# jianfch/stable-ts

Measured on AMD Instinct MI355X. Metric: real-time factor (audio-sec/wall-sec) large-v3 word_timestamps=True, higher is better.
Workload: dtype f16; 1 GPU; large-v3 (random-init, weight recipe BENCH_WEIGHTS = the parity-pinned recipe of tests/test_gpu_f16_depth.py), 10 min synthetic 16 kHz audio per GPU, word_timestamps=True, beam_size=5, 112 decode steps/window, window-parallel batch 20, default regrouping inside the timed pass; mode=transcribe, windows_per_gpu=20, segments=125, words=1670, parallelism=dp1 (windows sharded, no data-path collective)

## Files before the change

stable_ts_amd/csrc/swx_gemm.hip:

```cpp
#include <cstdlib>
#include <type_traits>
#include <array>
#include <vector>
#include <cstdio>
#include "swx_common.h"
#include "swx_kernels.h"

namespace {

template <typename T>
__device__ __forceinline__ void epilogue_store(const GemmArgs &g, int row, int col, float v)
{
    if (row >= g.M || col >= g.N) return;
    if (g.epi & EPI_BIAS) v += g.bias[col];
    if (g.epi & EPI_GELU) v = gelu_erf(v);
    if (g.epi & EPI_RESF32MOD) v += g.Rf[(size_t)(row % g.res_mod) * g.N + col];
    if (g.epi & EPI_RES) v += to_f32<T>(((const T *)g.R)[(size_t)row * g.ldr + col]);
    if (g.epi & EPI_STORE_VT) {
        const int w = row / g.vt_s, sidx = row - w * g.vt_s;
        ((T *)g.C)[(size_t)w * g.vt_bs + (size_t)col * g.vt_kp + sidx] = from_f32<T>(v);
    } else if (g.epi & EPI_CBATCH) {
        const int w = row / g.vt_s, sidx = row - w * g.vt_s;
        ((T *)g.C)[(size_t)w * g.vt_bs + (size_t)sidx * g.ldc + col] = from_f32<T>(v);
    } else if (g.epi & EPI_OUT_F32) ((float *)g.C)[(size_t)row * g.ldc + col] = v;
// ... 471 lines not shown
    for (int e = 0; e < 8; ++e) bv[e] = ((g.epi & EPI_BIAS) && gn + e < g.N) ? g.bias[gn + e] : 0.f;
#pragma unroll
    for (int p = 0; p < 4; ++p) {
        f16x8 rv[4];
        if (g.epi & EPI_RES) {
#pragma unroll
            for (int it = 0; it < 4; ++it) {
                const int gm = m0 + p * 64 + it * 16 + rb;
                rv[it] = (gm < g.M && full) ? *(const f16x8 *)((const f16 *)g.R + (size_t)gm * g.ldr + gn) : (f16x8)(f16)0;
            }
        }
        if (wm == (p >> 1)) {
#pragma unroll
            for (int ii = 0; ii < 4; ++ii)
#pragma unroll
                for (int j = 0; j < 4; ++j)
#pragma unroll
                    for (int r = 0; r < 4; ++r) Cs[ii * 16 + row_l + r][wn * 64 + j * 16 + col_l] = acc[(p & 1) * 4 + ii][j][r];
        }
        __syncthreads();
#pragma unroll
        for (int it = 0; it < 4; ++it) {
            const int row = it * 16 + rb, gm = m0 + p * 64 + row;
            if (gm >= g.M || !col_ok) continue;
            const f32x4 lo = *(const f32x4 *)&Cs[row][c8], hi = *(const f32x4 *)&Cs[row][c8 + 4];
            float v[8] = {lo[0], lo[1], lo[2], lo[3], hi[0], hi[1], hi[2], hi[3]};
#pragma unroll
            for (int e = 0; e < 8; ++e) v[e] += bv[e];
            if (g.epi & EPI_GELU) {
                gelu_erf_n<8>(v);
            }
            f16 *cp = (f16 *)g.C + (size_t)gm * g.ldc + gn;
            if (full) {
                if (g.epi & EPI_RES) {
#pragma unroll
                    for (int e = 0; e < 8; ++e) v[e] += (float)rv[it][e];
                }
                f16x8 o;
#pragma unroll
                for (int e = 0; e < 8; ++e) o[e] = (f16)v[e];
                *(f16x8 *)cp = o;
            } else {
                for (int e = 0; e < 8 && gn + e < g.N; ++e) {
                    float t = v[e];
                    if (g.epi & EPI_RES) t += (float)((const f16 *)g.R)[(size_t)gm * g.ldr + gn + e];
                    cp[e] = (f16)t;
                }
            }
        }
        if (p < 3) __syncthreads();
    }
}

constexpr int B8_HALF = 128 * 128;
constexpr int B8_BUF = 4 * B8_HALF;

template <int N>
__device__ __forceinline__ void b8_wait_vm()
{
    asm volatile("s_waitcnt vmcnt(%0)" ::"n"(N) : "memory");
}
__device__ __forceinline__ void b8_barrier()
{
    asm volatile("s_barrier" ::: "memory");
}
__device__ __forceinline__ void b8_wait_lds()
{
    asm volatile("s_waitcnt lgkmcnt(0)" ::: "memory");
}

__global__ __launch_bounds__(512) void gemm_f16_big8(GemmArgs g)
{
    extern __shared__ __attribute__((aligned(1024))) unsigned char ring[];
    const int tid = threadIdx.x, lane = tid & 63, wave = tid >> 6;
    const int wave_u = __builtin_amdgcn_readfirstlane(wave);
    const int wm = wave >> 2, wn = wave & 3;
    const int wm_u = wave_u >> 2;
    int bx = blockIdx.x, by = blockIdx.y;
    {
        const int gx = gridDim.x, gy = gridDim.y, nwg = gx * gy, orig = by * gx + bx;
        const int xcd = orig & 7, q = nwg >> 3, r = nwg & 7;
        const int wg = (xcd < r ? xcd * (q + 1) : r * (q + 1) + (xcd - r) * q) + (orig >> 3);
        if (g.tile_order != 1 || gx <= 4) { bx = wg % gx; by = wg / gx; }
        else {
            constexpr int GN = 4;
            const int nfull = gx / GN, per = GN * gy;
            const int grp = wg / per;
            if (grp < nfull) { const int rem = wg - grp * per; by = rem / GN; bx = grp * GN + (rem - by * GN); }
            else { const int gl = gx - nfull * GN, rem = wg - nfull * per; by = rem / gl; bx = nfull * GN + (rem - by * gl); }
        }
    }
    const int m0 = by * BG, n0 = bx * BG;
    const f16 *A = (const f16 *)g.A;
    const f16 *W = (const f16 *)g.W;

    f32x4 acc[8][4];
#pragma unroll
    for (int i = 0; i < 8; ++i)
#pragma unroll
        for (int j = 0; j < 4; ++j) acc[i][j] = (f32x4){0.f, 0.f, 0.f, 0.f};

    const f16 *sA[2][2], *sB[2][2];
#pragma unroll
    for (int h = 0; h < 2; ++h)
#pragma unroll
        for (int c = 0; c < 2; ++c) {
            const int lr = (wave * 2 + c) * 8 + (lane >> 3);
            const int slot = (lane & 7) ^ ((lr >> 1) & 7);
            const int ra = (lr >> 6) * 128 + h * 64 + (lr & 63);
            const int rb = (lr >> 5) * 64 + h * 32 + (lr & 31);
            const int gm = m0 + ra < g.M ? m0 + ra : g.M - 1;
            const int gn = n0 + rb < g.N ? n0 + rb : g.N - 1;
            sA[h][c] = A + (size_t)gm * g.lda + slot * 8;
            sB[h][c] = W + (size_t)gn * g.ldw + slot * 8;
        }
    typedef __attribute__((address_space(3))) void lds_void;
    const unsigned ring0 = (unsigned)(uintptr_t)(lds_void *)ring;
    auto issue = [&](int kt, auto which_c) {
        constexpr int which = decltype(which_c)::value;
        constexpr bool isA = which == 0 || which == 3;
        constexpr int h = which >= 2 ? 1 : 0;
        constexpr int off = (isA ? 0 : 2 * B8_HALF) + h * B8_HALF;
        const unsigned dst = ring0 + (kt & 1) * B8_BUF + off + wave_u * 2048;
#pragma unroll
// ... 29 lines not shown
        constexpr int ih = decltype(ih_c)::value, jh = decltype(jh_c)::value;
        __builtin_amdgcn_s_setprio(1);
#pragma unroll
        for (int kk = 0; kk < 2; ++kk)
#pragma unroll
            for (int i = 0; i < 4; ++i)
#pragma unroll
                for (int j = 0; j < 2; ++j)
                    acc[ih * 4 + i][jh * 2 + j] = __builtin_amdgcn_mfma_f32_16x16x32_f16(fa[i][kk], fb[j][kk], acc[ih * 4 + i][jh * 2 + j], 0, 0, 0);
        __builtin_amdgcn_s_setprio(0);
    };
    auto tile = [&](auto mode_c, int t) {
        constexpr int MODE = decltype(mode_c)::value;
        const int buf = t & 1;
        read_a(buf, 0);
        read_b(buf, 0, fb0);
        b8_wait_vm<MODE == 2 ? 2 : 8>();
        b8_barrier();
        b8_wait_lds();
        if (MODE < 2) issue(t + 1, I3());
        quad(I0(), I0(), fb0);
        b8_barrier();
        read_b(buf, 1, fb1);
        b8_wait_vm<MODE == 2 ? 0 : 8>();
        b8_barrier();
        b8_wait_lds();
        if (MODE == 0) issue(t + 2, I0());
        quad(I0(), I1(), fb1);
        b8_barrier();
        read_a(buf, 1);
        b8_barrier();
        b8_wait_lds();
        if (MODE == 0) issue(t + 2, I1());
        quad(I1(), I1(), fb1);
        b8_barrier();
        if (MODE == 0) b8_wait_vm<8>();
        if (MODE == 1) b8_wait_vm<4>();
        b8_barrier();
        if (MODE == 0) issue(t + 2, I2());
        quad(I1(), I0(), fb0);
        b8_barrier();
    };

    issue(0, I0()); issue(0, I1()); issue(0, I2()); issue(0, I3());
    issue(1, I0()); issue(1, I1()); issue(1, I2());
    b8_wait_vm<10>();
    b8_barrier();
    if (wm_u == 1) b8_barrier();
    int t = 0;
    for (; t < KT - 2; ++t) tile(I0(), t);
    tile(I1(), t);
    tile(I2(), t + 1);
    if (wm_u == 0) b8_barrier();
    big_tile_epilogue(g, ring, acc, m0, n0, tid, lane, wm, wn);
}

constexpr int BK32 = 16, LD32 = BK32 + 1;

template <int BMT, int BNT, int ST>
__global__ __launch_bounds__(256) void gemm_f32_tiled(GemmArgs g)
{
    constexpr int WN = BNT >= 128 ? 2 : 1, WM = 4 / WN;
    constexpr int WROWS = BMT / WM, WCOLS = BNT / WN;
    constexpr int NI = WROWS / 16, NJ = WCOLS / 16;
    constexpr int NA = (BMT * 4 + 255) / 256, NB = (BNT * 4 + 255) / 256;
    static_assert(NI >= 1 && NJ >= 1, "a wave owns at least one 16 x 16 fragment");
    __shared__ float As[2][BMT][LD32];
    __shared__ float Bs[2][BNT][LD32];
    const int tid = threadIdx.x, lane = tid & 63, wave = tid >> 6;
    const int wm = WN == 2 ? wave >> 1 : wave, wn = WN == 2 ? wave & 1 : 0;
    const int m0 = blockIdx.y * BMT, n0 = blockIdx.x * BNT;
    const float *A = (const float *)g.A;
    const float *W = (const float *)g.W;

    f32x4 acc[NI][NJ];
#pragma unroll
    for (int i = 0; i < NI; ++i)
#pragma unroll
        for (int j = 0; j < NJ; ++j) acc[i][j] = (f32x4){0.f, 0.f, 0.f, 0.f};

    f32x4 ra[ST][NA], rb[ST][NB];
    auto load_regs = [&](int st, int k0) {
#pragma unroll
        for (int i = 0; i < NA; ++i) {
            const int c = tid + 256 * i, row = c >> 2, kc = (c & 3) * 4;
            const int gm = m0 + row;
            ra[st][i] = (row < BMT && gm < g.M) ? *(const f32x4 *)(A + (size_t)gm * g.lda + k0 + kc) : (f32x4){0.f, 0.f, 0.f, 0.f};
        }
#pragma unroll
        for (int i = 0; i < NB; ++i) {
            const int c = tid + 256 * i, row = c >> 2, kc = (c & 3) * 4;
            const int gn = n0 + row;
            rb[st][i] = (row < BNT && gn < g.N) ? *(const f32x4 *)(W + (size_t)gn * g.ldw + k0 + kc) : (f32x4){0.f, 0.f, 0.f, 0.f};
        }
    };
    auto store_lds = [&](int st, int buf) {
#pragma unroll
        for (int i = 0; i < NA; ++i) {
            const int c = tid + 256 * i, row = c >> 2, kc = (c & 3) * 4;
            if (row < BMT) {
#pragma unroll
                for (int e = 0; e < 4; ++e) As[buf][row][kc + e] = ra[st][i][e];
            }
        }
#pragma unroll
        for (int i = 0; i < NB; ++i) {
            const int c = tid + 256 * i, row = c >> 2, kc = (c & 3) * 4;
            if (row < BNT) {
// ... 191 lines not shown
        const int m = t * 16 + fr;
        aok[t] = m < g.M;
        ap[t] = A + (size_t)(aok[t] ? m : 0) * g.lda + kb + fk;
    }
    f16x8 af[2][MT];
#pragma unroll
    for (int t = 0; t < MT; ++t) { const f16x8 v = *(const f16x8 *)(ap[t]); af[0][t] = aok[t] ? v : zero8; }
#pragma unroll
    for (int ks = 0; ks < NKS_MAX; ++ks) {
        if (ks < nks) {
            if (ks + 1 < nks) {
#pragma unroll
                for (int t = 0; t < MT; ++t) { const f16x8 v = *(const f16x8 *)(ap[t] + (ks + 1) * 32); af[(ks + 1) & 1][t] = aok[t] ? v : zero8; }
            }
#pragma unroll
            for (int t = 0; t < MT; ++t) acc[t] = __builtin_amdgcn_mfma_f32_16x16x32_f16(af[ks & 1][t], wf[ks], acc[t], 0, 0, 0);
        }
    }

    if (wave > 0) {
#pragma unroll
        for (int t = 0; t < MT; ++t) red[wave - 1][t][lane] = acc[t];
    }
    __syncthreads();
    if (wave == 0) {
        const int col = n0 + (lane & 15), row_l = (lane >> 4) * 4;
#pragma unroll
        for (int t = 0; t < MT; ++t) {
            f32x4 v = acc[t];
#pragma unroll
            for (int w = 0; w < 3; ++w) {
                const f32x4 o = red[w][t][lane];
                v[0] += o[0]; v[1] += o[1]; v[2] += o[2]; v[3] += o[3];
            }
#pragma unroll
            for (int r = 0; r < 4; ++r) epilogue_store<f16>(g, t * 16 + row_l + r, col, v[r]);
        }
    }
}

}

int swx_gemm_plan_f16(int M, int N, int K, int epi, int64_t ldc, int64_t ldr, bool ptr16, int force_kernel, int flags)
{
    if (K % 32 != 0) return -4;
    const bool skinny_ok = M <= 128 && K % 128 == 0 && K / 128 <= 10 && N <= 16384;
    if (force_kernel == 2) return skinny_ok ? SWX_GEMM_SKINNY : -4;
    if (skinny_ok && force_kernel != 1 && force_kernel < 7) return SWX_GEMM_SKINNY;
    const bool glds_ok = K % 64 == 0 && ptr16;
    if (force_kernel >= 7 && !glds_ok) return -4;
    if (force_kernel == 1 || !glds_ok) return SWX_GEMM_TILED_REG;
    const int64_t t128 = (int64_t)cdiv(N, BN) * cdiv(M, BM);
    const bool narrow = force_kernel == 8 || (force_kernel != 9 && N % 64 == 0 && t128 < 224);
    const bool big_ok = !(epi & ~(EPI_BIAS | EPI_GELU | EPI_RES)) && ldc % 8 == 0 && (!(epi & EPI_RES) || ldr % 8 == 0);
    if (force_kernel == 12) return big_ok && K >= 128 ? SWX_GEMM_BIG : -4;
    const int64_t t256 = (int64_t)cdiv(M, BG) * cdiv(N, BG);
    const double fill = (double)t256 / (double)(((t256 + 255) / 256) * 256);
    if (force_kernel == 0 && big_ok && t256 >= 200 && K >= 512 && (fill >= 0.9 || (fill >= 0.75 && K >= 2560)) &&
        !(flags & SWX_FLAG_NO_BIG_TILE))
        return SWX_GEMM_BIG;
    const bool ring_ok = K >= 128;
    if (force_kernel == 10 || force_kernel == 11) return !ring_ok ? -4 : force_kernel == 10 ? SWX_GEMM_RING64 : SWX_GEMM_RING128;
    if (force_kernel == 0 && ring_ok && M > 256 && (narrow || t128 <= 256) && !(flags & SWX_FLAG_NO_RING))
        return narrow ? SWX_GEMM_RING64 : SWX_GEMM_RING128;
    return narrow ? SWX_GEMM_GLDS64 : SWX_GEMM_GLDS128;
}

int swx_gemm(int dtype, const GemmArgs &g, int force_kernel, hipStream_t s)
{
    if (g.M <= 0 || g.N <= 0) return 0;
    if (dtype == SWX_F16) {
        if (g.lda % 8 != 0 || g.ldw % 8 != 0) return -4;
        const bool ptr16 = (uintptr_t)g.A % 16 == 0 && (uintptr_t)g.W % 16 == 0;
        const bool cr16 = (uintptr_t)g.C % 16 == 0 && (!(g.epi & EPI_RES) || (uintptr_t)g.R % 16 == 0);
        const int plan = swx_gemm_plan_f16(g.M, g.N, g.K, g.epi, cr16 ? g.ldc : 1, cr16 ? g.ldr : 1, ptr16, force_kernel, swx_flags());
        if (plan < 0) return plan;
        if (plan == SWX_GEMM_SKINNY) {
            SwxProfScope prof(PC_GEMM_SKINNY, 2.0 * ((double)g.N * g.K + (double)g.M * g.K) + (double)g.M * g.N * ((g.epi & EPI_OUT_F32) ? 4 : 2), s);
            dim3 grid(cdiv(g.N, 16));
            const int mt = cdiv(g.M, 16);
            switch (mt) {
                case 1: hipLaunchKernelGGL(gemm_f16_skinny<1>, grid, dim3(256), 0, s, g); break;
                case 2: hipLaunchKernelGGL(gemm_f16_skinny<2>, grid, dim3(256), 0, s, g); break;
                case 3: hipLaunchKernelGGL(gemm_f16_skinny<3>, grid, dim3(256), 0, s, g); break;
                case 4: hipLaunchKernelGGL(gemm_f16_skinny<4>, grid, dim3(256), 0, s, g); break;
                case 5: hipLaunchKernelGGL(gemm_f16_skinny<5>, grid, dim3(256), 0, s, g); break;
                case 6: hipLaunchKernelGGL(gemm_f16_skinny<6>, grid, dim3(256), 0, s, g); break;
                case 7: hipLaunchKernelGGL(gemm_f16_skinny<7>, grid, dim3(256), 0, s, g); break;
                default: hipLaunchKernelGGL(gemm_f16_skinny<8>, grid, dim3(256), 0, s, g); break;
            }
        } else {
            SwxProfScope prof(PC_GEMM_TILED, 2.0 * (double)g.M * g.N * g.K, s);
            const dim3 grid(cdiv(g.N, BN), cdiv(g.M, BM));
            switch (plan) {
                case SWX_GEMM_BIG: {
                    GemmArgs gb = g;
                    gb.tile_order = (swx_flags() & SWX_FLAG_BIG8_GROUPED) ? 1 : 0;
                    hipLaunchKernelGGL(gemm_f16_big8, dim3(cdiv(g.N, BG), cdiv(g.M, BG)), dim3(512), 2 * B8_BUF, s, gb); break;
                }
                case SWX_GEMM_RING64: launch_ring<64, 3>(g, s); break;
                case SWX_GEMM_RING128: launch_ring<128, 3>(g, s); break;
                case SWX_GEMM_GLDS64: hipLaunchKernelGGL(gemm_f16_glds_64, dim3(cdiv(g.N, 64), grid.y), dim3(256), 0, s, g); break;
                case SWX_GEMM_GLDS128: hipLaunchKernelGGL(gemm_f16_glds_128, grid, dim3(256), 0, s, g); break;
                default: hipLaunchKernelGGL(gemm_f16_tiled, grid, dim3(256), 0, s, g); break;
            }
        }
    } else {
        if (g.K % 16 != 0 || g.lda % 4 != 0 || g.ldw % 4 != 0) return -4;
        SwxProfScope prof(PC_GEMM_TILED, 2.0 * (double)g.M * g.N * g.K, s);
        if (g.M <= BM && g.N >= 256 && g.K % 64 == 0 && force_kernel != 8) {
            if (g.N >= 2560) hipLaunchKernelGGL((gemm_f32_rows64<2>), dim3(cdiv(g.N, 32), cdiv(g.M, 64)), dim3(256), 0, s, g);
            else hipLaunchKernelGGL((gemm_f32_rows64<1>), dim3(cdiv(g.N, 16), cdiv(g.M, 64)), dim3(256), 0, s, g);
        } else if (g.M <= BM && g.N >= 256) {
            if (g.N >= 2560) hipLaunchKernelGGL((gemm_f32_tiled<64, 32, 4>), dim3(cdiv(g.N, 32), cdiv(g.M, 64)), dim3(256), 0, s, g);
            else hipLaunchKernelGGL((gemm_f32_tiled<64, 16, 4>), dim3(cdiv(g.N, 16), cdiv(g.M, 64)), dim3(256), 0, s, g);
        } else {
            hipLaunchKernelGGL((gemm_f32_tiled<128, 128, 4>), dim3(cdiv(g.N, BN), cdiv(g.M, BM)), dim3(256), 0, s, g);
        }
    }
    SWX_CHECK_LAUNCH();
    return 0;
}
```

stable_ts_amd/csrc/swx_kernels.h:

```cpp
#pragma once
#include <hip/hip_runtime.h>
#include <stdint.h>
#include "../../include/swx.h"

#define EPI_BIAS 1
#define EPI_GELU 2
#define EPI_RES 4
#define EPI_OUT_F32 8
#define EPI_RESF32MOD 16
#define EPI_CBATCH 64
#define EPI_STORE_VT 32
#define EPI_KV 128

#define EPI_QKV_VT 256

struct GemmArgs {
    const void *A; int64_t lda;
    const void *W; int64_t ldw;
    const float *bias;
    const void *R; int64_t ldr;
    const float *Rf; int res_mod;
    void *C; int64_t ldc;
    void *C2;
    void *P; int64_t p_bs;
    int p_nkpad, p_vcol0;
    int M, N, K;
    int epi;
    int vt_s, vt_kp; int64_t vt_bs;
    int vt_zero_pad;
    int tile_order;
};
int swx_gemm(int dtype, const GemmArgs &g, int force_kernel, hipStream_t s);
enum { SWX_GEMM_TILED_REG = 0, SWX_GEMM_SKINNY = 1, SWX_GEMM_GLDS128 = 2, SWX_GEMM_GLDS64 = 3, SWX_GEMM_RING64 = 4, SWX_GEMM_RING128 = 5,
       SWX_GEMM_BIG = 6 };
int swx_gemm_plan_f16(int M, int N, int K, int epi, int64_t ldc, int64_t ldr, bool ptr16, int force_kernel, int flags);

#define SWX_FLAG_TABLE(X) \
    X(NO_FAST_STEP, 0)         \
    X(KCACHE_CHUNKED, 1)       \
    X(SELFATTN_NO_DEEP, 2)     \
    X(DEC_NO_W1, 4)            \
    X(TALL_NO_W8, 5)           \
    X(FLASH_NO_QB1, 6)         \
    X(XKV_PACK_SEPARATE, 7)    \
    X(SELFATTN_NO_MQ, 8)       \
    X(XQ_FULL_TILE, 9)         \
    X(DEC_W1_FULL_TILE, 10)    \
    X(NO_PACKED_XKV, 11)       \
    X(SELECT_MEM, 13)          \
    X(NO_GRAPH, 14)            \
    X(NO_PREFETCH, 15)         \
    X(NO_RING, 16)             \
    X(NO_BIG_TILE, 17)         \
    X(SCORE_TILED, 18)         \
    X(NO_TALL, 19)             \
    X(NO_FUSED_XQ, 20)         \
    X(TICKET, 21)              \
    X(BIG8_GROUPED, 22)        \
    X(XKV_TWO_LAUNCHES, 23)    \
    X(LOUDNESS_ONE_WG, 24)     \
    X(XATTN_R5, 25)            \
    X(FLASH_PIPELINED, 26)     \
    X(SELFATTN_WG5, 27)        \
    X(QKV_SEPARATE_VT, 28)
#define SWX_FLAG_DEFINE(name, bit) constexpr int SWX_FLAG_##name = 1 << (bit);
SWX_FLAG_TABLE(SWX_FLAG_DEFINE)
#undef SWX_FLAG_DEFINE
#define SWX_FLAG_IN_RANGE(name, bit) && (bit) >= 0 && (bit) <= 30
#define SWX_FLAG_OR(name, bit) | (int64_t(1) << (bit))
#define SWX_FLAG_SUM(name, bit) + (int64_t(1) << (bit))
static_assert(true SWX_FLAG_TABLE(SWX_FLAG_IN_RANGE), "SWX_FLAG_TABLE: a bit index outside 0..30");
static_assert((int64_t(0) SWX_FLAG_TABLE(SWX_FLAG_OR)) == (int64_t(0) SWX_FLAG_TABLE(SWX_FLAG_SUM)), "SWX_FLAG_TABLE: two switches share a bit");
#undef SWX_FLAG_IN_RANGE
#undef SWX_FLAG_OR
#undef SWX_FLAG_SUM
#define SWX_DEFAULT_FLAGS 0
int swx_flags();

struct KLayout { int sp, sh, sc; };
__host__ __device__ inline KLayout swx_klayout(int chunked, int n_ctx, int d)
{
    return chunked ? KLayout{8, 64 * n_ctx, 8 * n_ctx} : KLayout{d, 64, 8};
}
__host__ __device__ inline int swx_kidx(const KLayout &L, int pos, int h, int chunk) { return h * L.sh + chunk * L.sc + pos * L.sp; }

#define DEC_LN 1
#define DEC_GELU 2
#define DEC_RES 4
#define DEC_QKV 8
#define DEC_SLAB 16
#define DEC_TICKET 32
struct DecPrefetch {
    const void *base;
    int lines;
};
DecPrefetch swx_dec_prefetch_of(const void *packed_w, int M, int N, int K, int epi);

struct DecGemmArgs {
    const _Float16 *A; int64_t lda;
    const _Float16 *W; int64_t ldw;
    int M, N, K;
// ... 138 lines not shown
```

stable_ts_amd/csrc/swx_runtime.hip:

```cpp
#include <cmath>
#include <cstring>
#include <cstdio>
#include "swx_model.h"

namespace {

size_t add_slot(swx_model *m, size_t &cur, const std::string &name, int kind, int64_t rows, int64_t cols, int64_t dst_ld,
                size_t bytes, size_t base_off = (size_t)-1, size_t sub_off = 0)
{
    Slot s;
    s.kind = kind; s.rows = rows; s.cols = cols; s.dst_ld = dst_ld;
    if (base_off == (size_t)-1) { s.off = cur; cur = align_up(cur + bytes); }
    else s.off = base_off + sub_off;
    m->slots[name] = s;
    return s.off;
}

void build_layout(swx_model *m)
{
    const swx_dims &D = m->dims;
    const size_t e = m->esz;
    size_t cur = 0;
    auto mat = [&](const std::string &n, int64_t r, int64_t c) { return add_slot(m, cur, n, SK_MAT, r, c, c, (size_t)r * c * e); };
    auto vec = [&](const std::string &n, int64_t c) { return add_slot(m, cur, n, SK_VEC, 1, c, c, (size_t)c * 4); };
// ... 431 lines not shown
            n_valid[b] > 480000)
            return -2;
        lens[2 * b] = n_valid[b];
        lens[2 * b + 1] = n_total[b];
    }
    hipStream_t s = S(stream);
    int32_t *d_lens = m->Wp<int32_t>(m->L.h1);
    hipError_t e = hipMemcpyAsync(d_lens, lens.data(), lens.size() * 4, hipMemcpyHostToDevice, s);
    if (e == hipSuccess) e = hipStreamSynchronize(s);
    if (e != hipSuccess) return -100 - (int)e;
    return swx_mel_ragged_launch(d_pcm, d_lens, B, m->A<float>(m->o_hann), m->A<double2>(m->o_twiddle),
                                 m->A<float>(m->o_filters), m->dims.n_mels, d_mel, m->Wp<unsigned>(m->L.gmax), group, s);
}

int swx_log_mel_ragged(swx_model *m, const float *d_pcm, const int32_t *n_valid, const int32_t *n_total, int B,
                       float *d_mel, int per_item_max, void *stream)
{
    return swx_log_mel_ragged_grouped(m, d_pcm, n_valid, n_total, B, d_mel, per_item_max ? 1 : B, stream);
}

int swx_encode(swx_model *m, const float *d_mel, int B, void *d_xa, void *stream)
{
    if (!m || !m->arena || !m->ws) return -9;
    if (B <= 0) return 0;
    if (B > m->max_windows) return -8;
    const swx_dims &D = m->dims;
    const int d = D.n_audio_state, H = D.n_audio_head, S_ = D.n_audio_ctx;
    const size_t e = m->esz;
    hipStream_t s = S(stream);
    unsigned char *melT = m->ws + m->L.melT, *h1 = m->ws + m->L.h1;
    unsigned char *x = m->ws + m->L.x, *h = m->ws + m->L.h, *qkv = m->ws + m->L.qkv, *att = m->ws + m->L.att, *u = m->ws + m->L.u;
    const int rows = B * S_;
    if (D.n_audio_ctx != 1500) return -2;

    SWX_TRY(swx_mel_transpose(m->dtype, d_mel, B, D.n_mels, m->Cp, melT, s));
    SWX_TRY(swx_fill_zero(h1, (size_t)B * 3002 * d * e, s));
    for (int b = 0; b < B; ++b) {
        const unsigned char *a = melT + (size_t)b * 3002 * m->Cp * e;
        unsigned char *c = h1 + ((size_t)b * 3002 + 1) * d * e;
        SWX_TRY(swx_gemm(m->dtype, swx_gemm_args(a, m->Cp, m->arena + m->o_conv1_w, 3 * m->Cp, m->A<float>(m->o_conv1_b), c, d,
                                             3000, d, 3 * m->Cp, EPI_BIAS | EPI_GELU), 0, s));
    }
    for (int b = 0; b < B; ++b) {
        const unsigned char *a = h1 + (size_t)b * 3002 * d * e;
        GemmArgs g = swx_gemm_args(a, 2 * d, m->arena + m->o_conv2_w, 3 * d, m->A<float>(m->o_conv2_b), x + (size_t)b * S_ * d * e, d,
                               S_, d, 3 * d, EPI_BIAS | EPI_GELU | EPI_RESF32MOD);
        g.Rf = m->A<float>(m->o_enc_pos); g.res_mod = S_;
        SWX_TRY(swx_gemm(m->dtype, g, 0, s));
    }
    for (int l = 0; l < D.n_audio_layer; ++l) {
        const LayerW &w = m->enc[l];
        SWX_TRY(swx_layernorm(m->dtype, x, d, m->A<float>(w.ln1_g), m->A<float>(w.ln1_b), h, d, rows, d, s));
        const bool fuse_vt = m->dtype == SWX_F16 && d % 128 == 0 && S_ % 4 == 0 && !(g_debug_flags & SWX_FLAG_QKV_SEPARATE_VT) &&
                             swx_gemm_plan_f16(rows, 3 * d, d, EPI_BIAS, 3 * d, 1, true, 0, g_debug_flags) != SWX_GEMM_BIG;
        {
            GemmArgs gq = swx_gemm_args(h, d, m->arena + w.wqkv, d, m->A<float>(w.bqkv), qkv, 3 * d, rows, 3 * d, d, EPI_BIAS | (fuse_vt ? EPI_QKV_VT : 0));
            if (fuse_vt) { gq.C2 = u; gq.vt_s = S_; gq.vt_kp = SWX_VT_KP; gq.vt_bs = (int64_t)H * 64 * SWX_VT_KP; gq.vt_zero_pad = 1; }
            SWX_TRY(swx_gemm(m->dtype, gq, 0, s));
        }
        AttnArgs a{};
        a.q = qkv; a.ldq = 3 * d; a.k = qkv + (size_t)d * e; a.v = qkv + (size_t)2 * d * e; a.ldkv = 3 * d; a.o = att; a.ldo = d;
        a.k_bs = (int64_t)S_ * 3 * d; a.v_bs = a.k_bs; a.vt_kp = 0;
        a.B = B; a.H = H; a.nq = S_; a.nk = S_; a.q_rows_per_batch = S_;
        if (m->dtype == SWX_F16) {
            if (!fuse_vt) SWX_TRY(swx_transpose_v(a.v, 3 * d, a.v_bs, S_, u, SWX_VT_KP, (int64_t)H * 64 * SWX_VT_KP, B, H, s));
            a.v = u; a.vt_kp = SWX_VT_KP; a.v_bs = (int64_t)H * 64 * SWX_VT_KP;
        }
        SWX_TRY(swx_attention(m->dtype, a, 0, s));
        SWX_TRY(swx_gemm_residual(m, att, d, w.wo, w.bo, x, d, rows, d, d, s));
        SWX_TRY(swx_layernorm(m->dtype, x, d, m->A<float>(w.ln2_g), m->A<float>(w.ln2_b), h, d, rows, d, s));
        SWX_TRY(swx_gemm(m->dtype, swx_gemm_args(h, d, m->arena + w.w1, d, m->A<float>(w.b1), u, 4 * d, rows, 4 * d, d, EPI_BIAS | EPI_GELU), 0, s));
        SWX_TRY(swx_gemm_residual(m, u, 4 * d, w.w2, w.b2, x, d, rows, d, 4 * d, s));
    }
    SWX_TRY(swx_layernorm(m->dtype, x, d, m->A<float>(m->o_lnpost_g), m->A<float>(m->o_lnpost_b), d_xa, d, rows, d, s));
    return 0;
}

size_t swx_cross_kv_bytes(const swx_model *m, int B)
{
    if (!m) return 0;
    return (size_t)m->dims.n_text_layer * B * (size_t)xkv_chunk_elems(m) * m->esz;
}

int swx_cross_kv(swx_model *m, const void *d_xa, int B, void *d_xkv, void *stream)
{
    if (!m || !m->arena) return -9;
    const swx_dims &D = m->dims;
    const int d = D.n_text_state, S_ = D.n_audio_ctx;
    const size_t e = m->esz;
    if (D.n_audio_state != d) return -1;
    const int64_t chunk = xkv_chunk_elems(m);
    hipStream_t s = S(stream);
    SWX_TRY(swx_pad_zero((unsigned char *)d_xkv + (size_t)S_ * d * e, (int64_t)SWX_VT_KP * e, chunk * (int64_t)e, (int)(S_ * e),
                         (int)((SWX_VT_KP - S_) * e), d, D.n_text_layer * B, s));
    for (int l = 0; l < D.n_text_layer; ++l) {
        const LayerW &w = m->dec[l];
        unsigned char *base = (unsigned char *)d_xkv + (size_t)l * B * chunk * e;
        const bool one_launch = m->dtype == SWX_F16 && d % 128 == 0 && (int64_t)B * S_ > 128 && !(g_debug_flags & SWX_FLAG_XKV_TWO_LAUNCHES);
        bool packed_by_epilogue = false;
        if (one_launch) {
            GemmArgs gkv = swx_gemm_args(d_xa, d, m->arena + w.wckv, d, m->A<float>(w.bckv), base, d, B * S_, 2 * d, d, EPI_BIAS | EPI_KV);
            gkv.vt_s = S_; gkv.vt_kp = SWX_VT_KP; gkv.vt_bs = chunk; gkv.C2 = base + (size_t)S_ * d * e;
            if (!(g_debug_flags & SWX_FLAG_XKV_PACK_SEPARATE)) {
                gkv.P = base + (size_t)xkv_plain_elems(D) * e; gkv.p_bs = chunk; gkv.p_nkpad = ((S_ + 31) / 32) * 32; gkv.p_vcol0 = d;
                packed_by_epilogue = true;
            }
            SWX_TRY(swx_gemm(m->dtype, gkv, 0, s));
// ... 31 lines not shown
```

stable_ts_amd/csrc/swx_testhooks.hip:

```cpp
#include <cstring>
#include "swx_model.h"

__global__ __launch_bounds__(64) void lane_xor_check_kernel(const uint32_t *__restrict__ in, uint32_t *__restrict__ out)
{
    const int lane = threadIdx.x;
    const uint32_t x = in[blockIdx.x * 64 + lane];
    uint32_t *o = out + (size_t)blockIdx.x * 13 * 64 + lane;
    o[0 * 64] = lane_xor_u32<32>(x, lane); o[1 * 64] = lane_xor_u32<16>(x, lane); o[2 * 64] = lane_xor_u32<8>(x, lane);
    o[3 * 64] = lane_xor_u32<4>(x, lane);  o[4 * 64] = lane_xor_u32<2>(x, lane);  o[5 * 64] = lane_xor_u32<1>(x, lane);
    o[6 * 64] = (uint32_t)__shfl_xor((int)x, 32, 64); o[7 * 64] = (uint32_t)__shfl_xor((int)x, 16, 64);
    o[8 * 64] = (uint32_t)__shfl_xor((int)x, 8, 64);  o[9 * 64] = (uint32_t)__shfl_xor((int)x, 4, 64);
    o[10 * 64] = (uint32_t)__shfl_xor((int)x, 2, 64); o[11 * 64] = (uint32_t)__shfl_xor((int)x, 1, 64);
    double v = (double)__uint_as_float(x);
    double ref = v;
#pragma unroll
    for (int off = 32; off > 0; off >>= 1) ref += __shfl_xor(ref, off, 64);
    const double got = wave_sum_d(v);
    unsigned ok = (__double_as_longlong(got) == __double_as_longlong(ref)) ? 1u : 0u;
    const float f = (float)(int)(x >> 9) * 1.1920929e-7f - 0.37f;
    ok |= (__float_as_uint(lane_xor16_max(f)) == __float_as_uint(fmaxf(f, __shfl_xor(f, 16, 64)))) ? 2u : 0u;
    ok |= (__float_as_uint(lane_xor32_max(f)) == __float_as_uint(fmaxf(f, __shfl_xor(f, 32, 64)))) ? 4u : 0u;
    ok |= (__float_as_uint(lane_xor16_add(f)) == __float_as_uint(f + __shfl_xor(f, 16, 64))) ? 8u : 0u;
    ok |= (__float_as_uint(lane_xor32_add(f)) == __float_as_uint(f + __shfl_xor(f, 32, 64))) ? 16u : 0u;
    float wm = f, ws = f;
// ... 215 lines not shown
int swx_test_self_attn_plan(int dtype, int R, int H, int n_new, int n_ctx, int row_mul, int skip_append, int step_cached, int pos_bound,
                            int pos0_all_zero, int has_anc, int flags)
{
    static int32_t some_table;
    SelfAttnArgs sa{};
    sa.anc = has_anc ? &some_table : nullptr;
    sa.R = R; sa.n_new = n_new; sa.H = H; sa.n_ctx = n_ctx; sa.d = 64 * H; sa.skip_append = skip_append;
    sa.step_cached = step_cached; sa.pos_bound = pos_bound; sa.pos0_all_zero = pos0_all_zero;
    return swx_self_attn_plan(dtype, sa, row_mul, flags);
}

int swx_test_dec_plan(int M, int N, int K, int epilogue, int flags)
{
    int mt = 1, ks2 = 1;
    bool ticket = false;
    return swx_dec_kernel_plan(M, N, K, epilogue & 31, (epilogue & 64) ? 1 : 0, (epilogue & DEC_RES) != 0, flags, &mt, &ks2, &ticket);
}

int swx_test_layernorm(int dtype, const void *d_x, const float *d_g, const float *d_b, void *d_y, int rows, int d, void *stream)
{
    return swx_layernorm(dtype, d_x, d, d_g, d_b, d_y, d, rows, d, S(stream));
}

int swx_test_attention(int dtype, const void *d_q, int64_t ldq, const void *d_k, const void *d_v, int64_t ldkv, void *d_o,
                       int64_t ldo, int B, int H, int nq, int nk, int force_kernel, int vt_kp, void *stream)
{
    AttnArgs a{};
    a.q = d_q; a.ldq = ldq; a.k = d_k; a.v = d_v; a.ldkv = ldkv; a.o = d_o; a.ldo = ldo;
    a.k_bs = (int64_t)nk * ldkv; a.vt_kp = vt_kp;
    a.v_bs = vt_kp ? (int64_t)H * 64 * vt_kp : (int64_t)nk * ldkv;
    a.B = B; a.H = H; a.nq = nq; a.nk = nk; a.q_rows_per_batch = nq;
    return swx_attention(dtype, a, force_kernel, S(stream));
}

int swx_test_gemm_layout(int dtype, const void *d_a, int64_t lda, const void *d_w, int64_t ldw, const float *d_bias, const void *d_res,
                         const float *d_resf, int res_mod, void *d_c, int64_t ldc, void *d_c2, void *d_p, int64_t p_bs, int p_nkpad,
                         int p_vcol0, int vt_s, int vt_kp, int64_t vt_bs, int vt_zero_pad, int M, int N, int K, int epilogue,
                         int force_kernel, void *stream)
{
    if (dtype != SWX_F16 && dtype != SWX_F32) return -1;
    if (!d_a || !d_w || !d_c || M <= 0 || N <= 0 || K <= 0 || lda <= 0 || ldw < K) return -1;
    if ((epilogue & EPI_BIAS) && !d_bias) return -1;
    if ((epilogue & EPI_RES) && !d_res) return -1;
    if ((epilogue & EPI_RESF32MOD) && (!d_resf || res_mod <= 0)) return -1;
    const int layout = epilogue & (EPI_CBATCH | EPI_STORE_VT | EPI_KV | EPI_QKV_VT);
    if (layout && vt_s <= 0) return -1;
    if ((epilogue & (EPI_STORE_VT | EPI_KV | EPI_QKV_VT)) && vt_kp < vt_s) return -1;
    if (layout & (layout - 1)) return -2;
    if (epilogue & (EPI_KV | EPI_QKV_VT)) {
        if (dtype != SWX_F16 || !d_c2) return -2;
        if ((epilogue & EPI_KV) ? N % 2 != 0 : N % 3 != 0) return -2;
        const int split = (epilogue & EPI_KV) ? N / 2 : (N / 3) * 2;
        const bool ptr16 = (uintptr_t)d_a % 16 == 0 && (uintptr_t)d_w % 16 == 0;
        const int plan = swx_gemm_plan_f16(M, N, K, epilogue, 1, 1, ptr16, force_kernel, swx_flags());
        if (plan < 0) return plan;
        if (plan == SWX_GEMM_SKINNY || plan == SWX_GEMM_BIG) return -2;
        const int width = (plan == SWX_GEMM_GLDS64 || plan == SWX_GEMM_RING64) ? 64 : 128;
        if (split % width != 0) return -2;
        if (vt_s % 4 != 0 || vt_kp % 4 != 0 || vt_bs % 4 != 0 || M % 4 != 0) return -2;
    } else if (vt_zero_pad) return -2;
    if (d_p) {
        if (!(epilogue & EPI_KV) || ldc % 8 != 0 || vt_bs % 8 != 0 || p_bs % 8 != 0 || p_vcol0 != N / 2) return -2;
        if (p_nkpad != ((vt_s + 31) / 32) * 32 || (epilogue & (EPI_RES | EPI_GELU | EPI_OUT_F32 | EPI_RESF32MOD))) return -2;
    }
    GemmArgs g = swx_gemm_args(d_a, lda, d_w, ldw, d_bias, d_c, ldc, M, N, K, epilogue);
    g.R = d_res; g.ldr = ldc; g.Rf = d_resf; g.res_mod = res_mod > 0 ? res_mod : 1;
    g.C2 = d_c2; g.P = d_p; g.p_bs = p_bs; g.p_nkpad = p_nkpad; g.p_vcol0 = p_vcol0;
    g.vt_s = vt_s; g.vt_kp = vt_kp; g.vt_bs = vt_bs; g.vt_zero_pad = vt_zero_pad ? 1 : 0;
    return swx_gemm(dtype, g, force_kernel, S(stream));
}

int swx_test_xkv_pack(const void *d_k, const void *d_vt, void *d_packed, int B, int H, int nk, int ldk, int vt_kp, int64_t batch_stride,
                      void *stream)
{
    if (!d_k || !d_vt || !d_packed || B <= 0 || H <= 0 || nk <= 0) return -1;
    if (ldk < 64 * H || ldk % 8 != 0 || vt_kp % 8 != 0 || batch_stride % 8 != 0) return -2;
    return swx_xkv_pack(d_k, d_vt, d_packed, B, H, nk, ldk, vt_kp, batch_stride, S(stream));
}

int swx_test_attention_packed(const void *d_q, int64_t ldq, const void *d_k, const void *d_v, int64_t ldkv, int64_t k_bs, int64_t v_bs,
                              const void *d_packed, void *d_o, int64_t ldo, int B, int H, int nq, int nk, int vt_kp, int force_kernel,
                              const void *d_x, int64_t ldx, int fq_rows, const void *d_wq, const float *d_gamma, const float *d_beta,
                              const float *d_bias, void *d_scratch, size_t scratch_bytes, void *stream)
{
    if (!d_o || B <= 0 || H <= 0 || nq <= 0 || nk <= 0 || vt_kp <= 0) return -1;
    if (!d_packed && (!d_k || !d_v)) return -1;
    if (!d_wq && !d_q) return -1;
    if (vt_kp % 8 != 0 || vt_kp < ((nk + 31) / 32) * 32 || k_bs % 8 != 0 || v_bs % 8 != 0 || ldo < 64 * H) return -2;
    if (d_k && (ldkv < 64 * H || ldkv % 8 != 0)) return -2;
    hipStream_t s = S(stream);
    AttnArgs a{};
    a.q = d_q; a.ldq = ldq; a.k = d_k; a.v = d_v; a.ldkv = ldkv; a.o = d_o; a.ldo = ldo;
    a.k_bs = k_bs; a.v_bs = v_bs; a.vt_kp = vt_kp; a.kv_packed = d_packed;
    a.B = B; a.H = H; a.nq = nq; a.nk = nk; a.q_rows_per_batch = nq;
    if (d_wq) {
        const int d = 64 * H;
        if (!d_x || !d_gamma || !d_beta || !d_bias || !d_scratch) return -1;
        if (ldx < d || ldx % 8 != 0 || fq_rows < (B - 1) * nq + 1) return -2;
        if (scratch_bytes < align_up((size_t)d * d * 2) + 2 * align_up((size_t)d * 4)) return -8;
        unsigned char *p = (unsigned char *)d_scratch;
        f16 *wf = (f16 *)p; p += align_up((size_t)d * d * 2);
        float *c1 = (float *)p; p += align_up((size_t)d * 4);
        float *c2 = (float *)p;
        SWX_TRY(swx_fold_ln(d_wq, d_gamma, d_beta, d_bias, wf, c1, c2, d, d, s));
        a.fq_x = (const f16 *)d_x; a.fq_ldx = ldx; a.fq_rows = fq_rows; a.fq_w = wf; a.fq_c1 = c1; a.fq_c2 = c2; a.fq_k = d;
    } else if (ldq < 64 * H || ldq % 8 != 0) return -2;
    return swx_attention(SWX_F16, a, force_kernel, s);
}

int swx_test_xattn_plan(int B, int H, int nq, int nk, int vt_kp, int has_packed, int has_fq, int force_kernel, int flags)
// ... 34 lines not shown
```

Measured before the change: 1458 x real time.

## Add layout-aware epilogue to big 256x256 GEMM for fused QKV/KV transpose stores

Adds a templated variant of the big8 f16 GEMM whose epilogue stages results in LDS and writes either row-major K/Q pieces or transposed V (VT) layouts, including the packed cross-attention KV copies and zero padding. The planner now lets EPI_KV and EPI_QKV_VT GEMMs use the big-tile kernel, and the encoder enables the fused QKV+VT path even when the plain QKV GEMM would pick the big tile. Previously those cases either fell back to smaller tile kernels or skipped the VT fusion and ran a separate transpose. The cost is extra LDS for the staging buffer, a one-time attribute call, and a more complex epilogue with new alignment checks.

```diff
diff --git a/stable_ts_amd/csrc/swx_gemm.hip b/stable_ts_amd/csrc/swx_gemm.hip
--- a/stable_ts_amd/csrc/swx_gemm.hip
+++ b/stable_ts_amd/csrc/swx_gemm.hip
@@ -547,6 +547,129 @@
     }
 }
 
+constexpr int BG_HP = 2 * BG + 16;
+constexpr int BG_TP = 2 * BG + 32;
+constexpr int B8_LDS_F16 = BG * BG_TP;
+
+__device__ __forceinline__ void big_lane_bias(const GemmArgs &g, int n0, int lane, int wn, float (&bj)[4])
+{
+#pragma unroll
+    for (int j = 0; j < 4; ++j) {
+        const int gn = n0 + wn * 64 + j * 16 + (lane & 15);
+        bj[j] = ((g.epi & EPI_BIAS) && gn < g.N) ? g.bias[gn] : 0.f;
+    }
+}
+
+__device__ __forceinline__ unsigned big_pack2(f16 lo, f16 hi)
+{
+    typedef _Float16 f16x2 __attribute__((ext_vector_type(2)));
+    const f16x2 h = {lo, hi};
+    return __builtin_bit_cast(unsigned, h);
+}
+
+__device__ __forceinline__ void big_stage_rows_f16(const GemmArgs &g, unsigned char *ring, f32x4 (&acc)[8][4], int n0, int lane, int wm, int wn)
+{
+    float bj[4];
+    big_lane_bias(g, n0, lane, wn, bj);
+    const bool odd = lane & 1;
+    unsigned char *base = ring + (wm * 128 + (lane >> 4) * 4 + (odd ? 2 : 0)) * BG_HP + (wn * 64 + (lane & 14)) * 2;
+#pragma unroll
+    for (int i = 0; i < 8; ++i)
+#pragma unroll
+        for (int j = 0; j < 4; ++j) {
+            const float v[4] = {acc[i][j][0] + bj[j], acc[i][j][1] + bj[j], acc[i][j][2] + bj[j], acc[i][j][3] + bj[j]};
+            const unsigned p01 = big_pack2((f16)v[0], (f16)v[1]), p23 = big_pack2((f16)v[2], (f16)v[3]);
+            const unsigned recv = (unsigned)__builtin_amdgcn_update_dpp(0, (int)(odd ? p01 : p23), 0xB1, 0xF, 0xF, true);
+            const unsigned mine = odd ? p23 : p01;
+            const unsigned c0 = odd ? recv : mine, c1 = odd ? mine : recv;
+            unsigned char *p = base + i * 16 * BG_HP + j * 32;
+            *(unsigned *)p = (c0 & 0xffffu) | (c1 << 16);
+            *(unsigned *)(p + BG_HP) = (c0 >> 16) | (c1 & 0xffff0000u);
+        }
+}
+
+__device__ __forceinline__ void big_stage_cols_f16(const GemmArgs &g, unsigned char *ring, f32x4 (&acc)[8][4], int n0, int lane, int wm, int wn)
+{
+    float bj[4];
+    big_lane_bias(g, n0, lane, wn, bj);
+    unsigned char *base = ring + (wn * 64 + (lane & 15)) * BG_TP + (wm * 128 + (lane >> 4) * 4) * 2;
+#pragma unroll
+    for (int i = 0; i < 8; ++i)
+#pragma unroll
+        for (int j = 0; j < 4; ++j) {
+            const f16x4 o = {(f16)(acc[i][j][0] + bj[j]), (f16)(acc[i][j][1] + bj[j]), (f16)(acc[i][j][2] + bj[j]), (f16)(acc[i][j][3] + bj[j])};
+            *(f16x4 *)(base + j * 16 * BG_TP + i * 32) = o;
+        }
+}
+
+template <bool KV>
+__device__ __forceinline__ void big_store_rows_f16(const GemmArgs &g, const unsigned char *ring, int m0, int n0, int tid)
+{
+    const int c8 = (tid & 31) * 8, rb = tid >> 5, gn = n0 + c8;
+#pragma unroll 4
+    for (int it = 0; it < 16; ++it) {
+        const int row = it * 16 + rb, gm = m0 + row;
+        if (gm >= g.M) break;
+        const f16x8 o = *(const f16x8 *)(ring + row * BG_HP + c8 * 2);
+        if (KV) {
+            const int wb = gm / g.vt_s, key = gm - wb * g.vt_s;
+            *(f16x8 *)((f16 *)g.C + (size_t)wb * g.vt_bs + (size_t)key * g.ldc + gn) = o;
+            if (g.P) {
+                *(f16x8 *)xkv_packed_k_piece(g, wb, key, gn) = o;
+                if (key + 1 == g.vt_s)
+                    for (int kz = g.vt_s; kz < g.p_nkpad; ++kz) *(f16x8 *)xkv_packed_k_piece(g, wb, kz, gn) = (f16x8)(f16)0;
+            }
+        } else {
+            *(f16x8 *)((f16 *)g.C + (size_t)gm * g.ldc + gn) = o;
+        }
+    }
+}
+
+__device__ __forceinline__ void big_store_cols_f16(const GemmArgs &g, const unsigned char *ring, f16 *vt, int m0, int n0, int tid)
+{
+    const int rg = tid & 63, cq = tid >> 6, gm = m0 + rg * 4;
+    if (gm >= g.M) return;
+    const int wb = gm / g.vt_s, sidx = gm - wb * g.vt_s;
+    const bool last = sidx + 4 == g.vt_s;
+    const f16x4 z = {(f16)0.f, (f16)0.f, (f16)0.f, (f16)0.f};
+    f16 *cbase = vt + (size_t)wb * g.vt_bs + sidx;
+#pragma unroll 4
+    for (int k = 0; k < 32; ++k) {
+        const int col = cq + 8 * k, gn = n0 + col;
+        if (gn >= g.N) break;
+        const f16x4 o = *(const f16x4 *)(ring + col * BG_TP + rg * 8);
+        *(f16x4 *)(cbase + (size_t)gn * g.vt_kp) = o;
+        if (g.P) {
+            *(f16x4 *)xkv_packed_v_piece(g, wb, sidx, gn - g.p_vcol0) = o;
+            if (last)
+                for (int kz = g.vt_s; kz < g.p_nkpad; kz += 4) *(f16x4 *)xkv_packed_v_piece(g, wb, kz, gn - g.p_vcol0) = z;
+        }
+        if (g.vt_zero_pad && last)
+            for (int zp = 4; sidx + zp < g.vt_kp; zp += 4) *(f16x4 *)(cbase + (size_t)gn * g.vt_kp + zp) = z;
+    }
+}
+
+template <bool LAYOUT>
+__device__ __forceinline__ void big_epilogue(const GemmArgs &g, unsigned char *ring, f32x4 (&acc)[8][4], int m0, int n0, int tid, int lane,
+                                             int wm, int wn)
+{
+    if constexpr (!LAYOUT) big_tile_epilogue(g, ring, acc, m0, n0, tid, lane, wm, wn);
+    else {
+        const bool kv = g.epi & EPI_KV;
+        const int split = kv ? g.N >> 1 : (g.N / 3) * 2;
+        if (n0 >= split) {
+            big_stage_cols_f16(g, ring, acc, n0, lane, wm, wn);
+            __syncthreads();
+            big_store_cols_f16(g, ring, (f16 *)g.C2 - (size_t)split * g.vt_kp, m0, n0, tid);
+        } else {
+            big_stage_rows_f16(g, ring, acc, n0, lane, wm, wn);
+            __syncthreads();
+            if (kv) big_store_rows_f16<true>(g, ring, m0, n0, tid);
+            else big_store_rows_f16<false>(g, ring, m0, n0, tid);
+        }
+    }
+}
+
 constexpr int B8_HALF = 128 * 128;
 constexpr int B8_BUF = 4 * B8_HALF;
 
@@ -564,7 +687,8 @@
     asm volatile("s_waitcnt lgkmcnt(0)" ::: "memory");
 }
 
-__global__ __launch_bounds__(512) void gemm_f16_big8(GemmArgs g)
+template <bool LAYOUT>
+__device__ __forceinline__ void gemm_f16_big8_body(const GemmArgs &g)
 {
     extern __shared__ __attribute__((aligned(1024))) unsigned char ring[];
     const int tid = threadIdx.x, lane = tid & 63, wave = tid >> 6;
@@ -700,8 +824,11 @@
     tile(I1(), t);
     tile(I2(), t + 1);
     if (wm_u == 0) b8_barrier();
-    big_tile_epilogue(g, ring, acc, m0, n0, tid, lane, wm, wn);
-}
+    big_epilogue<LAYOUT>(g, ring, acc, m0, n0, tid, lane, wm, wn);
+}
+
+__global__ __launch_bounds__(512) void gemm_f16_big8(GemmArgs g) { gemm_f16_big8_body<false>(g); }
+__global__ __launch_bounds__(512) void gemm_f16_b8_layout(GemmArgs g) { gemm_f16_big8_body<true>(g); }
 
 constexpr int BK32 = 16, LD32 = BK32 + 1;
 
@@ -999,7 +1126,10 @@
     if (force_kernel == 1 || !glds_ok) return SWX_GEMM_TILED_REG;
     const int64_t t128 = (int64_t)cdiv(N, BN) * cdiv(M, BM);
     const bool narrow = force_kernel == 8 || (force_kernel != 9 && N % 64 == 0 && t128 < 224);
-    const bool big_ok = !(epi & ~(EPI_BIAS | EPI_GELU | EPI_RES)) && ldc % 8 == 0 && (!(epi & EPI_RES) || ldr % 8 == 0);
+    const int lay = epi & (EPI_KV | EPI_QKV_VT);
+    const bool lay_ok = !(flags & SWX_FLAG_BIG8_NO_LAYOUT) && !(epi & ~(EPI_BIAS | lay)) && ldc % 8 == 0 &&
+                        (lay == EPI_KV ? N % 2 == 0 && (N / 2) % BG == 0 : lay == EPI_QKV_VT && N % 3 == 0 && ((N / 3) * 2) % BG == 0);
+    const bool big_ok = lay ? lay_ok : !(epi & ~(EPI_BIAS | EPI_GELU | EPI_RES)) && ldc % 8 == 0 && (!(epi & EPI_RES) || ldr % 8 == 0);
     if (force_kernel == 12) return big_ok && K >= 128 ? SWX_GEMM_BIG : -4;
     const int64_t t256 = (int64_t)cdiv(M, BG) * cdiv(N, BG);
     const double fill = (double)t256 / (double)(((t256 + 255) / 256) * 256);
@@ -1020,7 +1150,16 @@
         if (g.lda % 8 != 0 || g.ldw % 8 != 0) return -4;
         const bool ptr16 = (uintptr_t)g.A % 16 == 0 && (uintptr_t)g.W % 16 == 0;
         const bool cr16 = (uintptr_t)g.C % 16 == 0 && (!(g.epi & EPI_RES) || (uintptr_t)g.R % 16 == 0);
-        const int plan = swx_gemm_plan_f16(g.M, g.N, g.K, g.epi, cr16 ? g.ldc : 1, cr16 ? g.ldr : 1, ptr16, force_kernel, swx_flags());
+        int plan = swx_gemm_plan_f16(g.M, g.N, g.K, g.epi, cr16 ? g.ldc : 1, cr16 ? g.ldr : 1, ptr16, force_kernel, swx_flags());
+        if (plan == SWX_GEMM_BIG && (g.epi & (EPI_KV | EPI_QKV_VT))) {
+            bool ok = g.C2 && (uintptr_t)g.C2 % 8 == 0 && g.vt_s > 0 && g.vt_s % 4 == 0 && g.vt_kp % 4 == 0 && g.vt_bs % 4 == 0 && g.M % 4 == 0;
+            if (g.epi & EPI_KV) ok = ok && g.vt_bs % 8 == 0;
+            if (g.P) ok = ok && (g.epi & EPI_KV) && (uintptr_t)g.P % 16 == 0 && g.p_bs % 8 == 0 && g.p_vcol0 == g.N / 2;
+            if (!ok) {
+                if (force_kernel == 12) return -4;
+                plan = swx_gemm_plan_f16(g.M, g.N, g.K, g.epi, 1, 1, ptr16, force_kernel, swx_flags() | SWX_FLAG_NO_BIG_TILE);
+            }
+        }
         if (plan < 0) return plan;
         if (plan == SWX_GEMM_SKINNY) {
             SwxProfScope prof(PC_GEMM_SKINNY, 2.0 * ((double)g.N * g.K + (double)g.M * g.K) + (double)g.M * g.N * ((g.epi & EPI_OUT_F32) ? 4 : 2), s);
@@ -1043,7 +1182,18 @@
                 case SWX_GEMM_BIG: {
                     GemmArgs gb = g;
                     gb.tile_order = (swx_flags() & SWX_FLAG_BIG8_GROUPED) ? 1 : 0;
-                    hipLaunchKernelGGL(gemm_f16_big8, dim3(cdiv(g.N, BG), cdiv(g.M, BG)), dim3(512), 2 * B8_BUF, s, gb); break;
+                    const dim3 gbig(cdiv(g.N, BG), cdiv(g.M, BG));
+                    if (g.epi & (EPI_KV | EPI_QKV_VT)) {
+                        static bool attr_done = false;
+                        if (!attr_done) {
+                            hipError_t e_ = hipFuncSetAttribute((const void *)gemm_f16_b8_layout, hipFuncAttributeMaxDynamicSharedMemorySize, B8_LDS_F16);
+                            if (e_ != hipSuccess) return -100 - (int)e_;
+                            attr_done = true;
+                        }
+                        hipLaunchKernelGGL(gemm_f16_b8_layout, gbig, dim3(512), B8_LDS_F16, s, gb);
+                    } else
+                        hipLaunchKernelGGL(gemm_f16_big8, gbig, dim3(512), 2 * B8_BUF, s, gb);
+                    break;
                 }
                 case SWX_GEMM_RING64: launch_ring<64, 3>(g, s); break;
                 case SWX_GEMM_RING128: launch_ring<128, 3>(g, s); break;
diff --git a/stable_ts_amd/csrc/swx_kernels.h b/stable_ts_amd/csrc/swx_kernels.h
--- a/stable_ts_amd/csrc/swx_kernels.h
+++ b/stable_ts_amd/csrc/swx_kernels.h
@@ -47,6 +47,7 @@
     X(XQ_FULL_TILE, 9)         \
     X(DEC_W1_FULL_TILE, 10)    \
     X(NO_PACKED_XKV, 11)       \
+    X(BIG8_NO_LAYOUT, 12)      \
     X(SELECT_MEM, 13)          \
     X(NO_GRAPH, 14)            \
     X(NO_PREFETCH, 15)         \
diff --git a/stable_ts_amd/csrc/swx_runtime.hip b/stable_ts_amd/csrc/swx_runtime.hip
--- a/stable_ts_amd/csrc/swx_runtime.hip
+++ b/stable_ts_amd/csrc/swx_runtime.hip
@@ -507,7 +507,8 @@
         const LayerW &w = m->enc[l];
         SWX_TRY(swx_layernorm(m->dtype, x, d, m->A<float>(w.ln1_g), m->A<float>(w.ln1_b), h, d, rows, d, s));
         const bool fuse_vt = m->dtype == SWX_F16 && d % 128 == 0 && S_ % 4 == 0 && !(g_debug_flags & SWX_FLAG_QKV_SEPARATE_VT) &&
-                             swx_gemm_plan_f16(rows, 3 * d, d, EPI_BIAS, 3 * d, 1, true, 0, g_debug_flags) != SWX_GEMM_BIG;
+                             (swx_gemm_plan_f16(rows, 3 * d, d, EPI_BIAS, 3 * d, 1, true, 0, g_debug_flags) != SWX_GEMM_BIG ||
+                              swx_gemm_plan_f16(rows, 3 * d, d, EPI_BIAS | EPI_QKV_VT, 3 * d, 1, true, 0, g_debug_flags) == SWX_GEMM_BIG);
         {
             GemmArgs gq = swx_gemm_args(h, d, m->arena + w.wqkv, d, m->A<float>(w.bqkv), qkv, 3 * d, rows, 3 * d, d, EPI_BIAS | (fuse_vt ? EPI_QKV_VT : 0));
             if (fuse_vt) { gq.C2 = u; gq.vt_s = S_; gq.vt_kp = SWX_VT_KP; gq.vt_bs = (int64_t)H * 64 * SWX_VT_KP; gq.vt_zero_pad = 1; }
diff --git a/stable_ts_amd/csrc/swx_testhooks.hip b/stable_ts_amd/csrc/swx_testhooks.hip
--- a/stable_ts_amd/csrc/swx_testhooks.hip
+++ b/stable_ts_amd/csrc/swx_testhooks.hip
@@ -291,10 +291,11 @@
         if ((epilogue & EPI_KV) ? N % 2 != 0 : N % 3 != 0) return -2;
         const int split = (epilogue & EPI_KV) ? N / 2 : (N / 3) * 2;
         const bool ptr16 = (uintptr_t)d_a % 16 == 0 && (uintptr_t)d_w % 16 == 0;
-        const int plan = swx_gemm_plan_f16(M, N, K, epilogue, 1, 1, ptr16, force_kernel, swx_flags());
+        const int64_t ldc16 = (uintptr_t)d_c % 16 == 0 ? ldc : 1;
+        const int plan = swx_gemm_plan_f16(M, N, K, epilogue, ldc16, 1, ptr16, force_kernel, swx_flags());
         if (plan < 0) return plan;
-        if (plan == SWX_GEMM_SKINNY || plan == SWX_GEMM_BIG) return -2;
-        const int width = (plan == SWX_GEMM_GLDS64 || plan == SWX_GEMM_RING64) ? 64 : 128;
+        if (plan == SWX_GEMM_SKINNY) return -2;
+        const int width = plan == SWX_GEMM_BIG ? 256 : (plan == SWX_GEMM_GLDS64 || plan == SWX_GEMM_RING64) ? 64 : 128;
         if (split % width != 0) return -2;
         if (vt_s % 4 != 0 || vt_kp % 4 != 0 || vt_bs % 4 != 0 || M % 4 != 0) return -2;
     } else if (vt_zero_pad) return -2;
```

After: 1457 x real time. About the same (-0.1%).
